# hkbharath/MARL-MASS

Hardware: AMD Instinct MI355X
Metric: agent-steps/sec (whole node), MASS CBF shield on, 65536 envs x 8 CAVs (higher is better)
Workload: dtype f64

## Files before the change

### marl-mass_amd/csrc/mm_kernels.hip

```cpp
#include <hip/hip_runtime.h>
#include <math.h>
#include <stdio.h>
#include <string.h>

#include <type_traits>

#include "mm_device.h"
#include "mm_div.h"
#include "mm_handle.h"
#define MM_COUNTS_FN __host__ __device__ inline
#include "../../include/mm_counts.h"
#include "../../include/mm_policy_wide.h"

using namespace mm;

struct DevCfg {
  int env_kind, shield, nsub, T, action_masking, auto_reset, obs_f64, N, E, debug_flags, n_hdv;
  double dt, collision_reward, high_speed_reward, headway_cost, headway_time, merging_lane_cost;
  double rs_lo, rs_hi, eta, tau;
  double inv_dt, rs_span, rs_ispan, rs_span2, rs_ispan2;
  int agent_reward;
  int steer_vel;
  int *err;
  int traffic_density, mixed_traffic, num_cav;
// ... 311 lines not shown
    const double a_lc = clipd(acc, kLcMinAcc, kLcMaxAcc);
    v.act_acc = lc_vehicle ? a_lc : acc;
  } else {
  if (v.crashed) { v.act_steer = 0; st_t = 0; v.act_acc = -1.0 * v.v; }
  if (v.v > kMaxSpeed) v.act_acc = fmin(v.act_acc, 1.0 * (kMaxSpeed - v.v));
  else if (v.v < -kMaxSpeed) v.act_acc = fmax(v.act_acc, 1.0 * (kMaxSpeed - v.v));
  if (lc_vehicle) v.act_acc = clipd(v.act_acc, kLcMinAcc, kLcMaxAcc);
  }
}

template <bool SEL = false>
MM_DEV int corner_flags(double x, double y, double sh, double ch, int lane) {
  double cx = x + (kCornerLen * mmm_cos_sum(MMM_CORNER_SIN, MMM_CORNER_COS, sh, ch));
  double cyL = y - (kCornerLen * mmm_sin_sum(MMM_CORNER_SIN, MMM_CORNER_COS, sh, ch)) + 0.01;
  double cyR = y - (kCornerLen * mmm_sin_sum(-MMM_CORNER_SIN, MMM_CORNER_COS, sh, ch)) + 0.01;
  double s = cx - lane_sx(lane);
  if constexpr (SEL && kCornerSelects) {
    const bool kb = lane == MM_LANE_KB0;
    double sn = 0.0;
    if (kb) sn = sin_f<true>(kSinePuls * s + kSinePhase);
    const double off = kb ? kSineAmp * sn : 0.0;
    const bool lon = (-kVehLength <= s) & (s < lane_len(lane) + kVehLength);
    const double rL0 = cyL - lane_sy(lane), rR0 = cyR - lane_sy(lane);
    const double rL = kb ? rL0 - off : rL0, rR = kb ? rR0 - off : rR0;
    return (!((fabs(rL) <= kLaneWidth / 2 + 0) & lon) ? 1 : 0) | (!((fabs(rR) <= kLaneWidth / 2 + 0) & lon) ? 2 : 0);
  }
  double off = (lane == MM_LANE_KB0) ? kSineAmp * sin_f<SEL>(kSinePuls * s + kSinePhase) : 0.0;
  bool lon = (-kVehLength <= s && s < lane_len(lane) + kVehLength);
  double rL = cyL - lane_sy(lane), rR = cyR - lane_sy(lane);
  if (lane == MM_LANE_KB0) { rL = rL - off; rR = rR - off; }
  return (!(fabs(rL) <= kLaneWidth / 2 + 0 && lon) ? 1 : 0) | (!(fabs(rR) <= kLaneWidth / 2 + 0 && lon) ? 2 : 0);
}
MM_DEV int pose_code(int lane, int nl, int off) { return lane | nl << 3 | off << 6; }

struct Cand {
  double x, y, h, gvx, cpsi, spsi;
  int lane;
  int pk;
};
template <int KIND, bool SHIELDED, bool CORNERS = SHIELDED, bool GENERAL = true, bool SINE = false>
MM_DEV Cand predict(const Veh &v, double steer, double st_t, double sh, double ch, double dt, bool sv = false, double *sine_out = nullptr) {
  Cand c;
  double ht = st_t, sb, cb;
  if constexpr (GENERAL) {
    if (__any(sv || st_t != st_t)) {
      double s2, c2;
      mmm_sincos(sv ? v.sang : steer, &s2, &c2);
      if (sv || st_t != st_t) ht = 1.0 / 2 * (s2 / c2);
    }
  }
  mmm_slip_sincos(ht, &sb, &cb);
  double vx = v.v * mmm_cos_sum(sh, ch, sb, cb), vy = v.v * mmm_sin_sum(sh, ch, sb, cb);
  c.x = v.x + vx * dt;
  c.y = v.y + vy * dt;
  const double d_heading = MM_DIVC(v.v * sb, 2.5);
  c.h = v.h + (sv ? d_heading : d_heading * dt);
  mmm_sincos(c.h, &c.spsi, &c.cpsi);
  c.gvx = (KIND == MM_ENV_V1) ? mmm_cos_sum(c.spsi, c.cpsi, sb, cb) : 0.0;
  c.lane = closest_lane<SINE>(c.x, c.y, c.h, sine_out);
  c.pk = c.lane;
  if (SHIELDED) c.pk = pose_code(c.lane, next_lane(c.lane, c.x, c.y), CORNERS ? corner_flags<SINE>(c.x, c.y, c.spsi, c.cpsi, c.lane) : 0);
  return c;
}

MM_DEV int adj_pair(int l1, int l2) {
  return (l1 == MM_LANE_BC0 && l2 == MM_LANE_BC1) ? -1 : ((l1 == MM_LANE_BC1 && l2 == MM_LANE_BC0) ? 1 : 0);
}
MM_DEV int adj_lane(int l1, int nl1, int l2) {
  const int f = adj_pair(l1, l2);
  return f != 0 ? f : adj_pair(nl1, l2);
}
MM_DEV unsigned adj_row(int l1) { return l1 == MM_LANE_BC0 ? (3u << (2 * MM_LANE_BC1)) : (l1 == MM_LANE_BC1 ? (1u << (2 * MM_LANE_BC0)) : 0u); }
MM_DEV unsigned adj_col(int l2) { return l2 == MM_LANE_BC1 ? (3u << (2 * MM_LANE_BC0)) : (l2 == MM_LANE_BC0 ? (1u << (2 * MM_LANE_BC1)) : 0u); }

struct QpTrace {
  double rows, a, h0, h1, h2, h3, d, margin;
};

MM_DEV void init_vehicle(Veh &v) {
  v.lane = closest_lane(v.x, v.y, v.h);
  v.tlane = v.lane;
  v.act_steer = v.act_acc = 0;
  v.safe_steer = v.safe_acc = 0;
  if (v.kind == 2) {
    v.sidx = 0;
    v.tspeed = v.v;
    v.gvx = py_mod((v.x + v.y) * kPi, 1.0);
  } else {
    v.sidx = speed_to_index(v.v);
    v.tspeed = index_to_speed(v.sidx);
    v.gvx = __builtin_nan("");
  }
  v.h1x = v.h1vx = v.h2x = v.h2vx = 0;
  v.sang = 0;
// ... 27 lines not shown
  else if (a < n_cav + n_sh) { main_road = true; k = n_s + (a - n_cav); }
  else { main_road = false; k = n_m + (a - n_cav - n_sh); }
  int slots[6];
#pragma unroll
  for (int i = 0; i < 6; i++) slots[i] = (main_road ? 10 : 5) + 50 * i;
  int chosen = 0;
#pragma unroll
  for (int i = 0; i < 6; i++) {
    if (i <= k) {
      const uint32_t ri = main_road ? r[i] : r[6 + i];
      int j = i + (int)(((uint64_t)ri * (uint32_t)(6 - i)) >> 32);
      int si = slots[i], sj = 0;
#pragma unroll
      for (int q = 0; q < 6; q++) if (q == j) sj = slots[q];
#pragma unroll
      for (int q = 0; q < 6; q++) if (q == j) slots[q] = si;
      slots[i] = sj;
      if (i == k) chosen = sj;
    }
  }
  rng_block(seed, episode, 3u + (uint32_t)a, blk);
  double speed = u53(blk[0], blk[1]) * 2 + 25;
  double noise = u53(blk[2], blk[3]) * 8 - 4;
  v.x = chosen + noise;
  v.y = main_road ? 0.0 : 10.5;
  v.h = 0;
  v.v = speed;
  v.kind = a < n_cav ? 1 : 2;
  v.present = true;
  init_vehicle(v);
  return n_m;
}

template <int G, int KIND, bool LEND = false, bool SEL = kScanSelects>
MM_DEV void observe(const DevCfg &c, const Veh &v, int a, int gb, long long i, bool valid, void *obs,
                    uint8_t *avail, float *stage = nullptr, const double *sincos_h = nullptr) {
  constexpr int F = (KIND != MM_ENV_V0) ? 6 : 5;
  constexpr int S = 5 * F;
  const bool ctrl = kIdm<KIND> ? v.present : (v.present && v.kind != 2);
  float *sw;
  if constexpr (LEND) {
    sw = stage + (threadIdx.x >> 6) * (64 * S);
  } else {
    __shared__ float s_obs[4][64 * S];
    sw = s_obs[threadIdx.x >> 6];
  }
  static_assert(64 * S * sizeof(float) >= 5 * 64 * sizeof(double), "the mailbox must fit in the row staging");
  if (obs) {
    const int lane = lane_id();
    double sps, cps;
    if (sincos_h) { sps = sincos_h[0]; cps = sincos_h[1]; }
    else mmm_sincos(v.h, &sps, &cps);
    const double vx = v.v * cps, vy = v.v * sps;
    const double sx = lane_sx(v.lane);
    double *mb = (double *)sw;
    mb[0 * 64 + lane] = v.x; mb[1 * 64 + lane] = v.y; mb[2 * 64 + lane] = vx; mb[3 * 64 + lane] = vy;
    if (KIND != MM_ENV_V0) mb[4 * 64 + lane] = v.h;
    __builtin_amdgcn_fence(__ATOMIC_RELEASE, "wavefront");
    __builtin_amdgcn_wave_barrier();
    __builtin_amdgcn_fence(__ATOMIC_ACQUIRE, "wavefront");
    double key[G];
    key[0] = 0;
    for_partners<G>([&](auto mc) {
      constexpr int m = decltype(mc)::value;
      const int pl = plane<m, G>(lane, a);
      double px = mb[0 * 64 + pl], py = mb[1 * 64 + pl];
      bool pp = px_i<m, G>((int)v.present, a) != 0;
// ... 58 lines not shown
      put(0, ctrl ? 1.0 : 0.0);
#pragma unroll
      for (int f = 0; f < F - 1; f++) {
        if constexpr (SEL) { const double w = lmap(ego[f], f); put(1 + f, ctrl ? w : 0.0); }
        else put(1 + f, ctrl ? lmap(ego[f], f) : 0.0);
      }
#pragma unroll
      for (int q = 0; q < 4; q++) {
        bool hq;
        if constexpr (SEL) hq = ctrl & have[q];
        else hq = ctrl && have[q];
        put((q + 1) * F, hq ? 1.0 : 0.0);
#pragma unroll
        for (int f = 0; f < F - 1; f++) {
          if constexpr (SEL) { const double w = lmap(row[q][f], f); put((q + 1) * F + 1 + f, hq ? w : 0.0); }
          else put((q + 1) * F + 1 + f, hq ? lmap(row[q][f], f) : 0.0);
        }
      }
    };
    if (c.obs_f64) {
      if (valid) emit([&](int k, double val) { ((double *)obs)[i * (5 * F) + k] = val; });
    } else {
      const int slot = (lane / G) * c.N + a;
      if (valid) emit([&](int k, double val) { sw[slot * S + k] = (float)val; });
      __builtin_amdgcn_fence(__ATOMIC_RELEASE, "wavefront");
      __builtin_amdgcn_wave_barrier();
      __builtin_amdgcn_fence(__ATOMIC_ACQUIRE, "wavefront");
      const long long wave_lane0 = (long long)blockIdx.x * blockDim.x + threadIdx.x - lane;
      const long long e0 = kPow2<G> ? wave_lane0 / G : (wave_lane0 >> 6) * (64 / G);
      long long nenv = (long long)c.E - e0;
      nenv = nenv < 0 ? 0 : (nenv > 64 / G ? 64 / G : nenv);
      const int total = (int)nenv * c.N * S;
      float *dst = (float *)obs + e0 * c.N * S;
      if constexpr (S % 2 == 0) {
        for (int t = lane; t < total / 2; t += 64) ((float2 *)dst)[t] = ((const float2 *)sw)[t];
      } else {
        for (int t = lane; t < total; t += 64) dst[t] = sw[t];
      }
    }
  }
  unsigned bits = 0x1F;
  if (!kIdm<KIND> && c.action_masking) {
    unsigned mine = 0;
    if (ctrl) {
      mine = 1u << 1;
      if (v.lane == MM_LANE_BC1 && lane_reachable(MM_LANE_BC0, v.x, v.y)) mine |= 1u << 0;
      if (v.lane == MM_LANE_BC0 && lane_reachable(MM_LANE_BC1, v.x, v.y)) mine |= 1u << 2;
      if (v.sidx < 4) mine |= 1u << 3;
      if (v.sidx > 0) mine |= 1u << 4;
    }
    bits = 0;
#pragma unroll
    for (int k = 0; k < 5; k++)
      if (group_ballot<G>((mine >> k) & 1u, gb)) bits |= 1u << k;
  }
  if (valid && avail) {
#pragma unroll
    for (int k = 0; k < 5; k++) avail[i * 5 + k] = (!kIdm<KIND> && ctrl) ? (uint8_t)((bits >> k) & 1u) : (uint8_t)0;
  }
}

struct Body {
  bool present, is_object;
  double x, y, h, v, tspeed;
  int lane;
  double sh, ch, koff;
};
MM_DEV double desired_gap(const Body &ego, const Body &front) {
  constexpr double ab = 15.0;
  const double es = ego.sh, ec = ego.ch, fs = front.sh, fc = front.ch;
// ... 188 lines not shown
  o.us0 = us0; o.veto = veto; o.flags = fl;
  o.qt.rows = s.cadj ? 4 : 3; o.qt.a = s.g0; o.qt.h0 = r.h0; o.qt.h1 = s.h1; o.qt.h2 = s.h2; o.qt.h3 = r.h3; o.qt.d = d;
  o.qt.margin = fmin(fmin(s.hls_lona, inv_lona), fmin(s.hls_lonr, inv_lonr));
  return o;
}
template <bool MASS, bool PRE = false, bool IPM = false>
MM_DEV ShieldOut shield_dyn(const DevCfg &c, const Veh &v, const ShieldStatic &s, const Neigh &nb, bool run_qp = true) {
  const ShieldRows r = shield_rows<PRE>(c, s, nb);
  double d;
  bool optimal = true;
  if constexpr (IPM) {
    d = 0.0;
    if (run_qp) {
      double slack;
      int iters;
      optimal = mm_qp_ipm_cbf(s.g0, r.h0, s.h1, s.h2, r.h3, s.cadj ? 4 : 3, &d, &slack, &iters) != 0;
    }
  } else {
    d = qp_exact(s, r);
  }
  return shield_post<MASS>(c, v, s, r, d, optimal, IPM && run_qp);
}
template <bool MASS, bool PRE = false, bool IPM = false>
MM_DEV ShieldOut shield_eval(const DevCfg &c, const Veh &v, double cpsi, int pk_self, const Neigh &nb, bool run_qp = true) {
  const ShieldStatic s = shield_static<MASS>(c, v, cpsi, pk_self, nb);
  return shield_dyn<MASS, PRE, IPM>(c, v, s, nb, run_qp);
}

struct Rel {
  double key;
  int cls;
  bool cflag;
};
MM_DEV Rel relate(double ex, double ey, int epk, bool other, double ox, double oy, double oh, int opk, bool o_hdv = false) {
  const int elane = epk & 7, enl = (epk >> 3) & 7, olane = opk & 7, onl = (opk >> 3) & 7;
  Rel r;
  const double dx = ox - ex, dy = oy - ey;
  const bool close = other & ((dx * dx + dy * dy) < kT180);
  const double esx = lane_sx(elane);
  const double ld = (ox - esx) - (ex - esx);
  r.key = close ? fabs(ld) : INFINITY;
  const unsigned rowE = adj_row(elane), rowN = adj_row(enl);
  const unsigned nzE = (rowE | rowE >> 1) & 0x555u;
  const unsigned rowEN = rowE | (rowN & ~(nzE * 3u));
  const unsigned colE = adj_col(elane);
  const unsigned va_c = (rowEN >> (2 * olane)) & 3u;
  const unsigned g1 = (colE >> (2 * olane)) & 3u, g2 = (colE >> (2 * onl)) & 3u;
  const unsigned av_c = g1 != 0 ? g1 : g2;
  const bool head = (dy < 0) ? (oh > 0.037) : (oh < -0.037);
  const bool appr = (!(ld < 0)) & (fabs(dy) <= 3.5) & head;
  const bool adj = (!appr) & ((va_c | av_c) != 0);
  const bool same = (elane == olane) | (olane == enl);
  const bool twin = o_hdv & (!adj) & (elane == MM_LANE_AB0) & (olane == MM_LANE_KB0) & (ld >= 0);
  const bool lead = (!adj) & (!twin) & (same | appr) & (ld > 0);
  const int cls = adj ? ((ld < 0) ? 3 : 2) : (twin ? 4 : (lead ? 1 : 0));
  r.cls = close ? cls : 0;
  r.cflag = ((opk >> (((va_c == 3u) | (av_c == 1u)) ? 6 : 7)) & 1) != 0;
  return r;
}

MM_DEV void trace_status(double *t, long long A, const ShieldOut &o) {
  t[MM_T_STATUS * A] = (double)(MM_ST_RAN | (o.optimal ? MM_ST_IS_OPTIMAL : 0u) | (o.lon_safe ? MM_ST_IS_SAFE : 0u) |
                                (o.lon_invariant ? MM_ST_IS_INVARIANT : 0u) | (o.bounds ? MM_ST_QP_BOUNDS : 0u));
  t[MM_T_HEADWAY * A] = o.hw_num / o.hw_den;
}

#ifndef MM_SWEEP_GATE_T
#define MM_SWEEP_GATE_T 48
#endif
#ifndef MM_SWEEP_GATE_W
#define MM_SWEEP_GATE_W 8
#endif
#ifndef MM_SWEEP_SPEC_AT
#define MM_SWEEP_SPEC_AT 13
#endif
#ifndef MM_SWEEP_GATE_WU
#define MM_SWEEP_GATE_WU 3
#endif
template <int NV, bool MASS, bool MIXED = false>
__global__ __launch_bounds__(64, 1) void sweep_kernel(DevCfg c, DevState st, SweepBuf sb, int k, double *trace) {
  const long long A = st.A;
  enum { W_X = 0, W_Y, W_H, W_HX, W_GU, W_VX };
// ... 372 lines not shown
#endif
__global__ __launch_bounds__(MM_STEP_BLOCK, (SPLIT ? MM_SPLIT_WAVES : step_min_waves<G, SHIELD, MIXED>(IPM))) void step_kernel(DevCfg c, DevState st, const int32_t *__restrict__ actions,
                                                   MMStepOut out, double *metrics, SweepBuf sb, int kb, PoseBuf pb) {
  constexpr bool IDM = kIdm<KIND>;
  constexpr bool LC = (KIND == MM_ENV_V1) || IDM;
  constexpr bool SHIELDED = LC && (SHIELD != MM_SHIELD_NONE);
  static_assert(!IDM || (MIXED && SHIELD == MM_SHIELD_NONE && !IPM && !SPLIT), "hdv-v1: general unshielded kernels only");
  constexpr bool MASS = (SHIELD == MM_SHIELD_MASS);
  static_assert(!IPM || SHIELDED, "the IPM mode lives in shielded kernels");
  static_assert(!SPLIT || IPM, "the split form exists for the interior-point kernels");
#ifdef MM_SERIAL_ALL
  constexpr bool kSerialOnly = true || IPM;
#else
#ifdef MM_SERIAL_MASS
  constexpr bool kSerialOnly = MIXED || MASS || IPM;
#else
  constexpr bool kSerialOnly = MIXED;
#endif
#endif
  constexpr bool kSine = SHIELDED && !SPLIT && !MIXED && !IPM && !kSerialOnly && kPow2<G> && G <= 8;
  constexpr bool kScan = kScanSelects && !MIXED && !TRACE;
#ifndef MM_CARRY_POSE
#define MM_CARRY_POSE 1
#endif
  constexpr bool kCarry = kSine && MM_CARRY_POSE != 0;
#ifndef MM_PRIMARY_PRIOR
#define MM_PRIMARY_PRIOR 1
#endif
  constexpr bool kPrimary = kSine && !TRACE && kVetoPrior && MM_PRIMARY_PRIOR != 0;
#ifndef MM_SINE_CARRY
#define MM_SINE_CARRY 0
#endif
  constexpr bool kSineCarry = kPrimary && MM_SINE_CARRY != 0;
  constexpr bool kEarly = kSine && MM_EARLY_LOADS != 0;
  double car_sn = __builtin_nan("");
  (void)car_sn;
  static_assert(kPow2<G> || MM_STEP_BLOCK == 64, "rotation layouts: one wave per workgroup");
  const long long gtid = (long long)blockIdx.x * blockDim.x + threadIdx.x;
  constexpr int kTail = kPow2<G> ? 64 : (64 / G) * G;
  const bool tail = lane_id() >= kTail;
  const int gb = kPow2<G> ? (lane_id() & ~(G - 1)) : (tail ? kTail - G : lane_id() - lane_id() % G);
  const int a = kPow2<G> ? (int)(gtid % G) : lane_id() - gb;
  const long long e = kPow2<G> ? gtid / G : (tail ? (long long)st.E : (gtid >> 6) * (64 / G) + lane_id() / G);
  const bool valid = e < st.E && a < st.N;
  const long long i = e * st.N + a;
  const long long A = st.A;
  const double dt = c.dt;

#ifdef MM_STAMPS
  const unsigned long long _rec_t0 = __builtin_amdgcn_s_memtime(), _rec_rt0 = __builtin_amdgcn_s_memrealtime();
  unsigned long long _t_last = __builtin_amdgcn_s_memtime(), _t_acc = 0;
#endif
  Veh v;
  const bool sv = MIXED && KIND == MM_ENV_V1 && c.steer_vel != 0;
  int steps = 0, time = 0, n_merge = 0, episode = 0;
  int car_code = 0;
  long long car_kx = 0, car_ky = 0, car_kh = 0;
  double car_s = 0.0, car_c = 1.0;
  int act_raw = 1;
  (void)act_raw;
  if constexpr (kEarly) {
    if (valid) act_raw = actions[i];
    if (e < st.E) { n_merge = st.I[MM_E_N_MERGE * st.E + e]; episode = st.I[MM_E_EPISODE * st.E + e]; }
  }
  if constexpr (kCarry) {
    if (valid) {
      car_kx = __double_as_longlong(pb.F[PB_KX * A + i]); car_ky = __double_as_longlong(pb.F[PB_KY * A + i]);
      car_kh = __double_as_longlong(pb.F[PB_KH * A + i]);
      car_s = pb.F[PB_SIN * A + i]; car_c = pb.F[PB_COS * A + i]; car_code = pb.code[i];
    }
  }
  load_veh(st, i, valid, v, sv);
  if (e < st.E) {
    steps = st.I[MM_E_STEPS * st.E + e]; time = st.I[MM_E_TIME * st.E + e];
  }
  if (!MIXED && v.kind == 2) v.kind = 1;
  if (IDM && v.present) v.kind = 2;
  const bool hdv = MIXED && v.kind == 2;
  const bool ctrl = IDM ? v.present : (v.present && !hdv);
  const bool ctrl_x = IDM ? false : ctrl;
  int action;
  if constexpr (kEarly) action = ctrl ? act_raw : 1;
  else action = (!IDM && valid && ctrl) ? actions[i] : 1;
  if ((unsigned)action > 4u) {
    if (!SPLIT || kb == 0) atomicOr(c.err, MM_LATCH_BAD_ACTION);
    action = 1;
  }
  const unsigned present_bits = group_ballot<G>(v.present, gb);
  const unsigned ctrl_bits = group_ballot<G>(ctrl, gb);
  const int n_veh = __popc(present_bits), n_ctrl = __popc(ctrl_bits);
  if (!SPLIT || kb == 0) steps += 1;

  double cpsi = 1.0, spsi = 0.0;
  double st_t = __builtin_nan("");
  int pk_self = v.lane;
  bool carried = false;
  if constexpr (kCarry) {
    const bool hit = car_kx == __double_as_longlong(v.x) && car_ky == __double_as_longlong(v.y) && car_kh == __double_as_longlong(v.h) &&
                     (car_code >> 8) == ((kPoseWritten >> 8) | (MASS ? 1 : 0)) && (car_code & 7) == v.lane;
    carried = !__any(v.present && !hit);
    if (carried && v.present) { spsi = car_s; cpsi = car_c; pk_self = car_code & 0xFF; }
  }
  if (!carried) {
    if (v.present) mmm_sincos(v.h, &spsi, &cpsi);
    if (SHIELDED && v.present) pk_self = pose_code(v.lane, next_lane(v.lane, v.x, v.y), MASS ? corner_flags<kSine>(v.x, v.y, spsi, cpsi, v.lane) : 0);
  }

  enum { C_B = 0, C_H1X = 8, C_H1VX, C_H2X, C_H2VX, C_SSTEER, C_SACC, C_TSPEED, C_A = 15, C_GU0 = 23, C_GU1 = 24, C_PRE = 25, C_MSGW = 29 };
  constexpr bool kMailbox = G <= 8 || !kPow2<G>;
  constexpr bool kPackMsg = !kPow2<G>;
  constexpr int kColdB = kMailbox ? (kPackMsg ? 29 : 30) : 25;
  constexpr bool kRoomy = false;
  constexpr int C_CPSI = kColdB + G - 1, C_GVX = C_CPSI + 1;
  constexpr int kColdN = !SHIELDED ? 15 : (kSerialOnly ? 23 : kColdB + G - 1 + (kRoomy ? 2 : 0));
  static_assert(kColdN * MM_STEP_BLOCK * 8 >= (MM_STEP_BLOCK / 64) * 64 * 30 * 4, "the obs staging must fit in the cold slots");
  __shared__ double s_cold[kColdN][MM_STEP_BLOCK];
  const int tid = threadIdx.x;
  auto cold_i = [&](int slot, int col) -> int & { return ((int *)&s_cold[slot][col])[0]; };
  if (LC) {
    s_cold[C_H1X][tid] = v.h1x; s_cold[C_H1VX][tid] = v.h1vx; s_cold[C_H2X][tid] = v.h2x; s_cold[C_H2VX][tid] = v.h2vx;
    s_cold[C_SSTEER][tid] = v.safe_steer; s_cold[C_SACC][tid] = v.safe_acc;
  }
  s_cold[C_TSPEED][tid] = v.tspeed;
  if constexpr (kEarly) {
    static_assert(kMailbox && !kPackMsg, "the high words of the pose-code and rank-word slots must be free");
    ((int *)&s_cold[C_PRE + 3][tid])[1] = n_merge; ((int *)&s_cold[C_MSGW][tid])[1] = episode;
  }
  if constexpr (kRoomy) { s_cold[C_CPSI][tid] = cpsi; s_cold[C_GVX][tid] = v.gvx; }
  auto CPSI = [&]() -> double { if constexpr (kRoomy) return s_cold[C_CPSI][tid]; else return cpsi; };
  auto GVX = [&]() -> double { if constexpr (kRoomy) return s_cold[C_GVX][tid]; else return v.gvx; };
  bool env_active = IDM ? n_veh > 0 : n_ctrl > 0;
  if constexpr (SPLIT) {
    if (kb > 0) env_active = e < st.E && sb.envf[e] != 0;
  }
  STAMP(0);
  const int k_lo = SPLIT ? (kb > 0 ? kb - 1 : 0) : 0, k_hi = SPLIT ? (kb < c.nsub ? kb : c.nsub - 1) : c.nsub - 1;
  for (int k = k_lo; k <= k_hi; k++) {
    const bool head = !SPLIT || k == kb, tail = !SPLIT || k != kb;
    const bool live = env_active && v.present;
    QpTrace qt = {0, __builtin_nan(""), __builtin_nan(""), __builtin_nan(""), __builtin_nan(""),
                  __builtin_nan(""), __builtin_nan(""), __builtin_nan("")};
    int rank = 0;
    if ((SHIELDED || MIXED) && head) {
      for_partners<G>([&](auto mc) {
        constexpr int m = decltype(mc)::value;
        double px = px_d<m, G>(v.x, a);
        bool pp = px_i<m, G>((int)live, a) != 0;
        if constexpr (kScan) rank += (pp & ((px > v.x) | ((px == v.x) & (pidx<m, G>(a) < a)))) ? 1 : 0;
        else rank += (pp && (px > v.x || (px == v.x && pidx<m, G>(a) < a))) ? 1 : 0;
      });
    }
    if (head) v.tspeed = s_cold[C_TSPEED][tid];
    if (live && !hdv && head) {
      if (time % c.nsub == 0) hl_act<KIND>(v, action);
    }
    const int tl_pre = v.tlane;
    if (live && !hdv && head) controlled_act<!MIXED && !kPrimary, kSine>(v, -1, sv, st_t);
    if (head) s_cold[C_TSPEED][tid] = v.tspeed;
    if constexpr (MIXED) { STAMP(1); }
    if constexpr (MIXED) {
      if (head && __any(hdv && live)) {
        const bool acting = hdv && live && !v.crashed;
        double koff = 0.0, koff_obst = 0.0;
        if (__any(acting && v.lane == MM_LANE_KB0)) {
          koff = kSineAmp * mmm_sin(kSinePuls * (v.x - lane_sx(MM_LANE_KB0)) + kSinePhase);
          koff_obst = kSineAmp * mmm_sin(kSinePuls * (kObstX - lane_sx(MM_LANE_KB0)) + kSinePhase);
        }
        Body self = {true, false, v.x, v.y, v.h, v.v, v.tspeed, v.lane, spsi, cpsi, koff};
        const double s_me = v.x - lane_sx(v.lane);
        NbSel n0 = {0, 0, -1, -1}, n1 = {0, 0, -1, -1};
        const LaneFrame lf0 = lane_frame(v.lane);
        if (acting && lane_after_end(v.tlane, v.x)) v.tlane = next_lane(v.tlane, v.x, v.y);
        const int my_tl = v.tlane;
        const bool lc_branch = v.lane != my_tl;
        const bool same_road = lane_road(v.lane) == lane_road(my_tl);
        const bool timer_due = !lc_branch && (1.0 < v.gvx);
        const int side = v.lane == MM_LANE_BC0 ? MM_LANE_BC1 : (v.lane == MM_LANE_BC1 ? MM_LANE_BC0 : -1);
        const bool try_mobil = acting && timer_due && side >= 0 && lane_reachable(side < 0 ? 0 : side, v.x, v.y);
        const int sl = side < 0 ? 0 : side;
        const double s_side = v.x - lane_sx(sl);
        const LaneFrame lf1 = lane_frame(sl);
        unsigned abort_mask = 0;
        for_partners<G>([&](auto mc) {
          constexpr int m = decltype(mc)::value;
          const int p = pidx<m, G>(a);
          const bool bp = px_i<m, G>((int)live, a) != 0;
          const double bx = px_d<m, G>(v.x, a), by = px_d<m, G>(v.y, a), bk = px_d<m, G>(koff, a);
          if (acting) {
            neighbour_update(lf0, s_me, bp, bx, by, bk, p, n0);
            if (try_mobil) neighbour_update(lf1, s_side, bp, bx, by, bk, p, n1);
// ... 49 lines not shown
          const bool changed = nxt != tl_post;
          tl_post = nxt;
          if (!__any(changed)) break;
        }
        if constexpr (MIXED) { STAMP(5); }
        if (acting) {
          v.tlane = tl_post;
          v.act_acc = clipd(acc_f0, -6.0, 6.0);
        }
      }
      if (head && live && (!hdv || !v.crashed)) steer_lane(v, sv && !hdv, st_t);
      if (head && hdv && live) v.gvx += dt;
    }
    bool first_B = false;
    if constexpr (kPrimary) {
      static_assert(!MIXED && !SPLIT, "kPrimary: no HDVs, no steer_vel, every launch a whole step");
      first_B = (c.debug_flags & 1) == 0 && live && v.hist_len >= 2 && (v.tlane != v.lane || v.crashed) && !(v.flags & MM_FLAG_IS_LC_SAFE);
      if (live) {
        const int tl_1 = v.tlane + (first_B ? v.lane - v.tlane : 0);
        const double steer = steering_control<kSine, kSineCarry>(v.x, v.y, v.h, v.v, tl_1, st_t, car_sn);
        v.act_steer = clipd(steer, -kPi / 3, kPi / 3);
        const double steer_1 = v.act_steer, st_t_1 = st_t;
        clip_actions<kSine>(v, LC, st_t);
        if (first_B) { v.act_steer = steer_1; st_t = st_t_1; }
      }
    } else {
      if (live && head) clip_actions<kSine>(v, LC && !hdv, st_t);
    }
    STAMP(1);
    Cand cA;
    memset(&cA, 0, sizeof cA);
    const bool shield_on = SHIELDED && live && !hdv && v.hist_len >= 2;
    if constexpr (kSineCarry) car_sn = __builtin_nan("");
    if (live && head) cA = predict<KIND, SHIELDED, MASS, MIXED, kSine>(v, v.act_steer, st_t, spsi, cpsi, dt, sv && !hdv, kSineCarry ? &car_sn : nullptr);
    auto park = [&](auto base_c, const Cand &cc, double steer) {
      constexpr int base = decltype(base_c)::value;
      if constexpr (SHIELDED) {
        s_cold[base + 0][tid] = cc.x; s_cold[base + 1][tid] = cc.y; s_cold[base + 2][tid] = cc.h;
        cold_i(base + 3, tid) = cc.pk; s_cold[base + 4][tid] = cc.cpsi; s_cold[base + 5][tid] = steer;
        s_cold[base + 6][tid] = cc.gvx; s_cold[base + 7][tid] = cc.spsi;
      }
    };
    auto park_at = [&](int base, const Cand &cc, double steer) {
      s_cold[base + 0][tid] = cc.x; s_cold[base + 1][tid] = cc.y; s_cold[base + 2][tid] = cc.h;
      cold_i(base + 3, tid) = cc.pk; s_cold[base + 4][tid] = cc.cpsi; s_cold[base + 5][tid] = steer;
      s_cold[base + 6][tid] = cc.gvx; s_cold[base + 7][tid] = cc.spsi;
    };
    if constexpr (kPrimary) park_at(first_B ? (int)C_B : (int)C_A, cA, v.act_steer);
    else if (head) park(std::integral_constant<int, C_A>{}, cA, v.act_steer);
    STAMP(2);
    const bool needB = SHIELDED && shield_on && (v.tlane != v.lane || v.crashed || sv);
    bool haveB = first_B, haveA = !first_B;
    (void)haveA;
    auto make_other = [&]() {
      if constexpr (kPrimary) {
        const bool mk_A = !haveA;
        if (mk_A || (needB && !haveB)) {
          double t_o;
          const int tl_o = v.lane + (mk_A ? v.tlane - v.lane : 0);
          double steer_o = steering_control<kSine>(v.x, v.y, v.h, v.v, tl_o, t_o);
          if (mk_A) {
            steer_o = clipd(steer_o, -kPi / 3, kPi / 3);
            if (v.crashed) { steer_o = 0; t_o = 0; }
          }
          park_at(mk_A ? (int)C_A : (int)C_B, predict<KIND, true, MASS, MIXED, kSine>(v, steer_o, t_o, spsi, cpsi, dt, false), steer_o);
          haveA = true; haveB = haveB || !mk_A;
        }
      }
    };
    auto make_B = [&]() {
      if constexpr (SHIELDED) {
        if (needB && !haveB) {
          double tB;
          double steerB = steering_control<kSine>(v.x, v.y, v.h, v.v, v.lane, tB);
          if (sv) steerB = steer_vel_command(steerB, v.sang);
          park(std::integral_constant<int, C_B>{}, predict<KIND, true, MASS, MIXED, kSine>(v, steerB, tB, spsi, CPSI(), dt, sv), steerB);
          haveB = true;
        }
      }
    };
    auto chosen = [&](bool useB) {
      if constexpr (!SHIELDED) {
        return cA;
      } else {
        const int base = useB ? C_B : C_A;
        Cand cc;
        cc.x = s_cold[base + 0][tid]; cc.y = s_cold[base + 1][tid]; cc.h = s_cold[base + 2][tid];
        cc.gvx = s_cold[base + 6][tid]; cc.cpsi = s_cold[base + 4][tid]; cc.spsi = s_cold[base + 7][tid];
        const int pk = cold_i(base + 3, tid);
        cc.pk = pk; cc.lane = pk & 7;
        return cc;
      }
    };
    if constexpr (SPLIT) {
      if (!head && live && valid) {
        v.act_acc = sw_f(sb, SW_ACCN, a, e);
        if (MIXED && hdv) {
          v.act_steer = sw_f(sb, SW_ASTEER, a, e);
          if (sw_i(sb, SW_RES, a, e) & 16) s_cold[C_H1X][tid] = sw_f(sb, SW_ACC, a, e);
        }
        s_cold[C_A + 0][tid] = sw_f(sb, SW_AX, a, e); s_cold[C_A + 1][tid] = sw_f(sb, SW_AY, a, e); s_cold[C_A + 2][tid] = sw_f(sb, SW_AH, a, e);
        cold_i(C_A + 3, tid) = sw_i(sb, SW_APK, a, e); s_cold[C_A + 4][tid] = sw_f(sb, SW_ACPSI, a, e); s_cold[C_A + 5][tid] = sw_f(sb, SW_ASTEER, a, e);
        s_cold[C_A + 6][tid] = sw_f(sb, SW_AGVX, a, e); s_cold[C_A + 7][tid] = sw_f(sb, SW_ASPSI, a, e);
        if (needB) {
          s_cold[C_B + 0][tid] = sw_f(sb, SW_BX, a, e); s_cold[C_B + 1][tid] = sw_f(sb, SW_BY, a, e); s_cold[C_B + 2][tid] = sw_f(sb, SW_BH, a, e);
          cold_i(C_B + 3, tid) = sw_i(sb, SW_BPK, a, e); s_cold[C_B + 4][tid] = sw_f(sb, SW_BCPSI, a, e); s_cold[C_B + 5][tid] = sw_f(sb, SW_BSTEER, a, e);
          s_cold[C_B + 6][tid] = sw_f(sb, SW_BGVX, a, e); s_cold[C_B + 7][tid] = sw_f(sb, SW_BSPSI, a, e);
          haveB = true;
        }
// ... 69 lines not shown
          if ((threadIdx.x & 63) == 13) _t_acc += 1 + (pass == 0 ? 1ull << 32 : 0ull);
#endif
#endif
          const double mine_gvx = s_cold[(use_B ? C_B : C_A) + 6][tid];
          const double h1vx_mine = s_cold[C_H1VX][tid];
          s_cold[C_GU0][tid] = slot_gu<MASS>(s_cold[C_H2VX][tid], MASS ? s_cold[C_SACC][tid] : kCbfAccLo, GVX(), dt);
          s_cold[C_GU1][tid] = slot_gu<MASS>(h1vx_mine, kCbfAccLo, mine_gvx, dt);
          if constexpr (kMailbox) {
            const int my_word = (live ? rank : 99) | (use_B ? 256 : 0);
            if constexpr (kPackMsg) ((int *)&s_cold[C_PRE + 3][tid])[1] = my_word;
            else cold_i(C_MSGW, tid) = my_word;
            __builtin_amdgcn_fence(__ATOMIC_RELEASE, "wavefront");
            __builtin_amdgcn_wave_barrier();
            __builtin_amdgcn_fence(__ATOMIC_ACQUIRE, "wavefront");
          }
          Cand mine;
          if constexpr (!kMailbox) mine = chosen(use_B);
          double k_ol = INFINITY, k_oa = INFINITY, k_oar = INFINITY;
          int j_ol = -1, j_oa = -1, j_oar = -1;
          for_partners<G>([&](auto mc) {
            constexpr int m = decltype(mc)::value;
            const int p = pidx<m, G>(a);
            int p_rank, opk;
            double ox, oy, oh;
            bool i_first;
            if constexpr (kMailbox) {
              const int pl = plane<m, G>(tid, a);
              int pw;
              if constexpr (kPackMsg) pw = ((const int *)&s_cold[C_PRE + 3][pl])[1];
              else pw = cold_i(C_MSGW, pl);
              p_rank = pw & 255;
              i_first = live && rank < p_rank;
              const int pb = (!i_first && p_rank < 99) ? ((pw & 256) ? (int)C_B : (int)C_A) : (int)C_PRE;
              ox = s_cold[pb + 0][pl]; oy = s_cold[pb + 1][pl]; oh = s_cold[pb + 2][pl];
              opk = cold_i(pb + 3, pl) | (p_rank < 99 ? 256 : 0);
            } else {
              p_rank = dppx_i<m>(live ? rank : 99);
              i_first = live && rank < p_rank;
              const double sx_ = i_first ? mine.x : v.x, sy_ = i_first ? mine.y : v.y, sh_ = i_first ? mine.h : v.h;
              const int spk = i_first ? mine.pk : pk_self;
              ox = dppx_d<m>(sx_); oy = dppx_d<m>(sy_); oh = dppx_d<m>(sh_);
              opk = dppx_i<m>(spk | (int)live << 8);
            }
            const bool o_first = !i_first && p_rank < 99;
            const Rel r = relate(v.x, v.y, pk_self, ((opk >> 8) & 1) != 0, ox, oy, oh, opk);
            if constexpr (count5) s_cold[kColdB + m - 1][tid] = r.key;
            const bool b_ol = (r.cls == 1) & ((r.key < k_ol) | ((r.key == k_ol) & (p < (j_ol & 15))));
            const bool b_oa = (r.cls == 2) & ((r.key < k_oa) | ((r.key == k_oa) & (p < (j_oa & 15))));
            const bool b_oar = (r.cls == 3) & ((r.key < k_oar) | ((r.key == k_oar) & (p < (j_oar & 15))));
            const int pf = p | (o_first ? 16 : 0) | (r.cflag ? 32 : 0);
            k_ol = b_ol ? r.key : k_ol; j_ol = b_ol ? pf : j_ol;
            k_oa = b_oa ? r.key : k_oa; j_oa = b_oa ? pf : j_oa;
            k_oar = b_oar ? r.key : k_oar; j_oar = b_oar ? pf : j_oar;
          });
          const bool ol_first = j_ol >= 0 && (j_ol & 16), oa_first = j_oa >= 0 && (j_oa & 16), oar_stepped = j_oar >= 0 && (j_oar & 16);
          const bool cadj = j_oa >= 0 && (j_oa & 32);
          j_ol = j_ol < 0 ? -1 : (j_ol & 15); j_oa = j_oa < 0 ? -1 : (j_oa & 15); j_oar = j_oar < 0 ? -1 : (j_oar & 15);
          STAMP(3);
          Neigh nb;
          memset(&nb, 0, sizeof nb);
          nb.has_ol = j_ol >= 0; nb.has_oa = j_oa >= 0; nb.has_oar = j_oar >= 0;
          if constexpr (count5) {
            int pos_ol = 0, pos_oa = 0, pos_oar = 0;
#pragma unroll
            for (int m = 1; m < G; m++) {
              const int p = pidx_rt<G>(a, m);
              const double km = s_cold[kColdB + m - 1][tid];
              pos_ol += (km < k_ol || (km == k_ol && p < j_ol)) ? 1 : 0;
              pos_oa += (km < k_oa || (km == k_oa && p < j_oa)) ? 1 : 0;
              pos_oar += (km < k_oar || (km == k_oar && p < j_oar)) ? 1 : 0;
            }
            nb.has_ol = nb.has_ol && pos_ol < 5;
            nb.has_oa = nb.has_oa && pos_oa < 5;
            nb.has_oar = nb.has_oar && pos_oar < 5;
          }
          nb.constrain_adj = MASS && nb.has_oa && cadj;
          if constexpr (SPLIT) {
            if (valid && shield_on)
              sw_i(sb, SW_CLS, a, e) = (j_ol & 15) | (j_oa & 15) << 4 | (j_oar & 15) << 8 | (nb.has_ol ? 1 << 12 : 0) | (nb.has_oa ? 1 << 13 : 0) |
                                       (nb.has_oar ? 1 << 14 : 0) | (nb.constrain_adj ? 1 << 15 : 0);
            break;
          }
          __builtin_amdgcn_fence(__ATOMIC_RELEASE, "wavefront");
          __builtin_amdgcn_wave_barrier();
          __builtin_amdgcn_fence(__ATOMIC_ACQUIRE, "wavefront");
          const int t_ol = tid - a + (j_ol < 0 ? a : j_ol), t_oa = tid - a + (j_oa < 0 ? a : j_oa);
          nb.ol_x = s_cold[ol_first ? C_H1X : C_H2X][t_ol]; nb.ol_gu = s_cold[ol_first ? C_GU1 : C_GU0][t_ol];
          nb.oa_x = s_cold[oa_first ? C_H1X : C_H2X][t_oa]; nb.oa_gu = s_cold[oa_first ? C_GU1 : C_GU0][t_oa];
          const int src_ol = gb + (j_ol < 0 ? 0 : j_ol), src_oa = gb + (j_oa < 0 ? 0 : j_oa), src_oar = gb + (j_oar < 0 ? 0 : j_oar);
          const double cpsi_now = CPSI();
          nb.oar_x = shfl_d(v.x, src_oar); nb.oar_vx = shfl_d(v.v * cpsi_now, src_oar);
          bool ol_dyn = MASS && nb.has_ol && ol_first, oa_dyn = MASS && nb.has_oa && oa_first;
          {
            unsigned rep = obstacle_override<MASS>(nb, v.x, v.y);
            if (rep & 1u) ol_dyn = false;
            if (rep & 2u) oa_dyn = false;
          }
          irregular = irregular || (shield_on && nb.has_oar && oar_stepped);
          double acc_cur = shield_on ? 0.0 : v.act_acc;
          if constexpr (kRoomy) v.gvx = GVX();
          const ShieldStatic ss = shield_static<MASS>(c, v, cpsi_now, pk_self, nb);
          if constexpr (IPM) {
            bool fin = !shield_on, run = false, sing = false;
            bool late = false, late_opt = false;
            const bool slow_lc = MASS && (v.hl == 2 || v.hl == 0) && v.v < kStoppingSpeed;
            MMQpState q;
            q.x0 = 0.0; q.m4 = 0; q.iters = 0;
            bool more = true;
            for (int trip = 0; more; trip++) {
              if (trip > (MM_QP_MAXITERS + 2) * (G + 1)) { atomicOr(c.err, MM_LATCH_INTERNAL); break; }
              MMQpRes rs;
              bool done_now = late, opt = late_opt;
              late = false;
              if (run) {
                const int stop = mm_qp_top(&q, &rs);
                if (stop || sing) { run = false; done_now = true; opt = stop == 1 && !sing; }
              }
              if (__any(done_now)) {
                if (done_now) {
                  double us0 = ss.u0 + q.x0;
                  if (MASS && slow_lc) us0 = shield_post<MASS>(c, v, ss, shield_rows<true>(c, ss, nb), q.x0, opt, true).us0;
                  acc_cur = div_c(us0 - ss.evx, dt, c.inv_dt);
                  fin = true;
                  qc_d = q.x0; qc_meta = (ss.cadj ? 4 : 3) | (opt ? 8 : 0);
                }
              }
              bool ready = shield_on && !fin && !run;
              double da = 0.0, db = 0.0;
              if (MASS) {
                const double gu_cur = slot_gu<true>(h1vx_mine, acc_cur, mine_gvx, dt);
                da = shfl_d(gu_cur, src_ol); db = shfl_d(gu_cur, src_oa);
                const unsigned long long fm = __ballot(fin);
                ready = ready && (!ol_dyn || ((fm >> src_ol) & 1ull)) && (!oa_dyn || ((fm >> src_oa) & 1ull));
              }
// ... 172 lines not shown
            if constexpr (G >= 8) red(std::integral_constant<int, 7>{});
            if constexpr (G >= 16) red(std::integral_constant<int, 8>{});
          } else {
            auto ring = [&](auto mc) {
              constexpr int off = decltype(mc)::value;
              if constexpr (off < G) {
                const unsigned o = (unsigned)px_i<off, G>((int)w, a);
                const unsigned m0 = min(w & 0x3FFu, o & 0x3FFu), m1 = min((w >> 10) & 0x3FFu, (o >> 10) & 0x3FFu),
                               m2 = min((w >> 20) & 0x3FFu, (o >> 20) & 0x3FFu);
                w = m0 | m1 << 10 | m2 << 20;
                if (MIXED) f_tw = min(f_tw, (unsigned)px_i<off, G>((int)f_tw, a));
              }
            };
            ring(std::integral_constant<int, 1>{}); ring(std::integral_constant<int, 2>{});
            ring(std::integral_constant<int, 4>{}); ring(std::integral_constant<int, 8>{});
          }
          f_ol = w & 0x3FFu; f_oa = (w >> 10) & 0x3FFu; f_oar = (w >> 20) & 0x3FFu;
          const bool has_tw = MIXED && f_tw != none;
          if (has_tw) f_oa = f_tw & ~1u;
          Neigh nb;
          nb.has_ol = f_ol != none; nb.has_oa = f_oa != none; nb.has_oar = f_oar != none;
          const int s_ol = gb + (nb.has_ol ? (int)((f_ol >> 1) & 15u) : 0);
          const int s_oa = gb + (nb.has_oa ? (int)((f_oa >> 1) & 15u) : 0);
          const int s_oar = gb + (nb.has_oar ? (int)((f_oar >> 1) & 15u) : 0);
          nb.ol_x = shfl_d(whx, s_ol); nb.ol_gu = shfl_d(wgu, s_ol);
          nb.oa_x = shfl_d(whx, s_oa); nb.oa_gu = shfl_d(wgu, s_oa);
          nb.ol_vx = nb.oa_vx = nb.ol_acc = nb.ol_g = nb.oa_acc = nb.oa_g = 0;
          nb.oar_x = shfl_d(wx, s_oar); nb.oar_vx = shfl_d(wvx, s_oar);
          nb.constrain_adj = MASS && nb.has_oa && (f_oa & 1u);
          bool hss_collab = false;
          if (has_tw) { nb.constrain_adj = MASS; hss_collab = !MASS; }
          obstacle_override<MASS>(nb, v.x, v.y);
          const bool mine = has && a == ai && shield_on;
          ShieldOut s1 = shield_eval<MASS, true, IPM>(c, v, cpsi, pk_self, nb, mine);
          if (hss_collab) s1.flags |= MM_FLAG_IS_COLLABORATING;
          if (IPM && mine && s1.bounds) atomicOr(c.err, MM_LATCH_QP_BOUNDS);
          if (mine) {
            new_acc = s1.acc; veto = s1.veto; new_flags = s1.flags; qt = s1.qt;
            if (TRACE) trace_status(out.trace + (long long)k * MM_T_COUNT * A + i, A, s1);
            use_B = veto && needB;
            const Cand cc = chosen(use_B);
            double nv = v.v + new_acc * dt;
            nv = nv > 0 ? nv : 0;
            wx = cc.x; wy = cc.y; wh = cc.h; wg = cc.gvx; wacc = new_acc; wvx = nv * cc.cpsi;
            whx = s_cold[C_H1X][tid]; whvx = s_cold[C_H1VX][tid]; wpk = cc.pk;
            wgu = slot_gu<MASS>(whvx, MASS ? wacc : kCbfAccLo, wg, dt);
          }
        }
        if (MIXED && hdv && twin_shift != 0 && w_stepped) s_cold[C_H1X][tid] = whx;
      }
     }
    }
    STAMP(6);
    CAND_COUNT(MM_CS_PRIOR_HELD, st_prior && use_B);
    CAND_COUNT(MM_CS_PRIOR_LIFTED, st_prior && !use_B);
    if (SPLIT && SHIELDED && out.trace && live && tail && !shield_on) {
      out.trace[(long long)k * MM_T_COUNT * A + i + MM_T_QP_ROWS * A] = 0;
    }
    if (!SPLIT && SHIELDED && TRACE && live) {
      double *t = out.trace + (long long)k * MM_T_COUNT * A + i;
      t[MM_T_QP_ROWS * A] = qt.rows; t[MM_T_QP_A * A] = qt.a;
      t[MM_T_QP_H0 * A] = qt.h0; t[MM_T_QP_H1 * A] = qt.h1; t[MM_T_QP_H2 * A] = qt.h2;
      t[MM_T_QP_H3 * A] = qt.h3; t[MM_T_QP_D * A] = qt.d; t[MM_T_LC_MARGIN * A] = qt.margin;
    }
    if (tail) {
    if constexpr (kSineCarry) {
      if (!(live && use_B == first_B)) car_sn = __builtin_nan("");
// ... 289 lines not shown
        row[ln] = acc;
      }
    }
  }
  STAMP(15);
  if constexpr (kCarry) { car_s = spsi; car_c = cpsi; }
  if (c.auto_reset && done) {
    const uint64_t seed = st.seeds[e];
    Veh nv;
    memset(&nv, 0, sizeof nv);
    int nm = 0;
    int nc = n_ctrl, nh = n_veh - n_ctrl;
    if constexpr (IDM) { nc = 0; nh = n_veh; }
    episode_counts<KIND>(c, seed, (uint32_t)episode, nc, nh);
    const bool spawn = valid && (c.traffic_density > 0 ? a < nc + nh : v.present);
    if (spawn) nm = spawn_vehicle(nv, a, nc, nh, seed, (uint32_t)episode);
    if (c.traffic_density > 0 && valid) {
      if (!spawn) {
        if (v.present) {
          Veh z;
          memset(&z, 0, sizeof z);
          store_veh(st, i, z, true);
        }
        v.present = false; v.kind = 0;
      }
      st.B[MM_B_KIND * A + i] = spawn ? (uint8_t)nv.kind : (uint8_t)0;
    }
    if (spawn) {
      v = nv;
      spsi = 0.0; cpsi = 1.0;
      if constexpr (kCarry) {
        mmm_sincos(v.h, &car_s, &car_c);
        pk_self = pose_code(v.lane, next_lane(v.lane, v.x, v.y), MASS ? corner_flags<kSine>(v.x, v.y, car_s, car_c, v.lane) : 0);
      }
      s_cold[C_H1X][tid] = v.h1x; s_cold[C_H1VX][tid] = v.h1vx; s_cold[C_H2X][tid] = v.h2x; s_cold[C_H2VX][tid] = v.h2vx;
      s_cold[C_SSTEER][tid] = v.safe_steer; s_cold[C_SACC][tid] = v.safe_acc; s_cold[C_TSPEED][tid] = v.tspeed;
    }
    n_merge = shfl_i(nm, gb);
    steps = 0; time = 0; episode += 1;
  }
  if (valid && v.present) {
    if (LC) {
      v.h1x = s_cold[C_H1X][tid]; v.h1vx = s_cold[C_H1VX][tid]; v.h2x = s_cold[C_H2X][tid]; v.h2vx = s_cold[C_H2VX][tid];
      if (!hdv) { v.safe_steer = s_cold[C_SSTEER][tid]; v.safe_acc = s_cold[C_SACC][tid]; }
    }
    v.tspeed = s_cold[C_TSPEED][tid];
    store_veh(st, i, v, sv);
    if constexpr (kCarry) {
      pb.F[PB_KX * A + i] = v.x; pb.F[PB_KY * A + i] = v.y; pb.F[PB_KH * A + i] = v.h;
      pb.F[PB_SIN * A + i] = car_s; pb.F[PB_COS * A + i] = car_c;
      pb.code[i] = (pk_self & 0xFF) | (MASS ? 0x100 : 0) | kPoseWritten;
    }
  }
  if (e < st.E && a == 0) {
    st.I[MM_E_STEPS * st.E + e] = steps; st.I[MM_E_TIME * st.E + e] = time;
    st.I[MM_E_N_MERGE * st.E + e] = n_merge; st.I[MM_E_EPISODE * st.E + e] = episode;
  }
  STAMP(11);
  __syncthreads();
  STAMP(14);
  const double sc_h[2] = {spsi, cpsi};
  observe<G, KIND, true, kScan>(c, v, a, gb, i, valid, out.obs, out.action_mask, (float *)&s_cold[0][0], sc_h);
  STAMP(12);
#ifdef MM_STAMPS
  {
    const long long wv = gtid >> 6;
    if ((threadIdx.x & 63) < 16 && wv < MM_STAMP_WAVES) g_stamps_w[wv * 16 + (threadIdx.x & 63)] += _t_acc;
    else if ((threadIdx.x & 63) < 32 && wv < MM_STAMP_WAVES) g_stamps_c[wv * 16 + (threadIdx.x & 63) - 16] += _t_acc;
    if (wv < MM_REC_WAVES) {
      unsigned long long *rec = g_wave_rec + wv * MM_REC_WORDS;
      const int respawned = __popcll(__ballot(c.auto_reset && done && a == 0 && e < st.E));
      if ((threadIdx.x & 63) < 32) rec[MM_REC_SLOTS + (threadIdx.x & 63)] = _t_acc;
      if ((threadIdx.x & 63) == 0) {
        const unsigned hw = __builtin_amdgcn_s_getreg(4 | (31 << 11)), xcc = __builtin_amdgcn_s_getreg(20 | (31 << 11));
        rec[MM_REC_BEGIN] = _rec_t0; rec[MM_REC_RT_BEGIN] = _rec_rt0;
        rec[MM_REC_HW] = (unsigned long long)hw | (unsigned long long)xcc << 32;
        rec[MM_REC_RESPAWN] = (unsigned long long)respawned;
        rec[MM_REC_RT_END] = __builtin_amdgcn_s_memrealtime();
        rec[MM_REC_END] = __builtin_amdgcn_s_memtime();
      }
    }
  }
#endif
}

template <int G, int KIND>
__global__ __launch_bounds__(256) void reset_kernel(DevCfg c, DevState st, int mode, const uint8_t *env_mask,
                                                    const uint64_t *seeds_in, void *obs, uint8_t *avail) {
  const long long gtid = (long long)blockIdx.x * blockDim.x + threadIdx.x;
  const long long e = gtid / G;
  const int a = (int)(gtid % G);
  const int gb = lane_id() & ~(G - 1);
  const bool valid = e < st.E && a < st.N;
  const long long i = e * st.N + a;
  const bool selected = e < st.E && mode != 2 && (!env_mask || env_mask[e]);
// ... 1183 lines not shown
```

Before: 2.600 billion.

## Pack heading-sign bits into pose code, widen obs copy, branch-free action select

Three separate changes. First, the heading-threshold sign is encoded as two extra bits in the pose code, so the neighbour relate step no longer needs to load the other vehicle's heading from shared memory. Second, the observation copy from LDS staging to global uses unrolled float4 loads and stores when a wave's env block is full and aligned, with the old float2 loop kept as fallback. Third, the high-level and controlled action updates run unconditionally on a copy and are merged back with selects, trading extra work on idle lanes for less divergence.

Measured after the change: 2.640 billion, median of 6. 1.5% higher.

```diff
diff --git a/marl-mass_amd/csrc/mm_kernels.hip b/marl-mass_amd/csrc/mm_kernels.hip
--- a/marl-mass_amd/csrc/mm_kernels.hip
+++ b/marl-mass_amd/csrc/mm_kernels.hip
@@ -367,13 +367,19 @@
   return (!(fabs(rL) <= kLaneWidth / 2 + 0 && lon) ? 1 : 0) | (!(fabs(rR) <= kLaneWidth / 2 + 0 && lon) ? 2 : 0);
 }
 MM_DEV int pose_code(int lane, int nl, int off) { return lane | nl << 3 | off << 6; }
+#ifndef MM_POSE_HBITS
+#define MM_POSE_HBITS 1
+#endif
+constexpr bool kPoseHBits = MM_POSE_HBITS != 0;
+constexpr int kPoseHPos = 0x200, kPoseHNeg = 0x400;
+MM_DEV int pose_hbits(double h) { return ((h > 0.037) ? kPoseHPos : 0) | ((h < -0.037) ? kPoseHNeg : 0); }
 
 struct Cand {
   double x, y, h, gvx, cpsi, spsi;
   int lane;
   int pk;
 };
-template <int KIND, bool SHIELDED, bool CORNERS = SHIELDED, bool GENERAL = true, bool SINE = false>
+template <int KIND, bool SHIELDED, bool CORNERS = SHIELDED, bool GENERAL = true, bool SINE = false, bool HB = false>
 MM_DEV Cand predict(const Veh &v, double steer, double st_t, double sh, double ch, double dt, bool sv = false, double *sine_out = nullptr) {
   Cand c;
   double ht = st_t, sb, cb;
@@ -395,6 +401,7 @@
   c.lane = closest_lane<SINE>(c.x, c.y, c.h, sine_out);
   c.pk = c.lane;
   if (SHIELDED) c.pk = pose_code(c.lane, next_lane(c.lane, c.x, c.y), CORNERS ? corner_flags<SINE>(c.x, c.y, c.spsi, c.cpsi, c.lane) : 0);
+  if constexpr (HB) c.pk |= pose_hbits(c.h);
   return c;
 }
 
@@ -488,7 +495,11 @@
   return n_m;
 }
 
-template <int G, int KIND, bool LEND = false, bool SEL = kScanSelects>
+#ifndef MM_OBS_WIDE
+#define MM_OBS_WIDE 1
+#endif
+constexpr bool kObsWide = MM_OBS_WIDE != 0;
+template <int G, int KIND, bool LEND = false, bool SEL = kScanSelects, bool WIDE = false>
 MM_DEV void observe(const DevCfg &c, const Veh &v, int a, int gb, long long i, bool valid, void *obs,
                     uint8_t *avail, float *stage = nullptr, const double *sincos_h = nullptr) {
   constexpr int F = (KIND != MM_ENV_V0) ? 6 : 5;
@@ -613,10 +624,32 @@
       nenv = nenv < 0 ? 0 : (nenv > 64 / G ? 64 / G : nenv);
       const int total = (int)nenv * c.N * S;
       float *dst = (float *)obs + e0 * c.N * S;
-      if constexpr (S % 2 == 0) {
-        for (int t = lane; t < total / 2; t += 64) ((float2 *)dst)[t] = ((const float2 *)sw)[t];
+      auto copy_loop = [&]() {
+        if constexpr (S % 2 == 0) {
+          for (int t = lane; t < total / 2; t += 64) ((float2 *)dst)[t] = ((const float2 *)sw)[t];
+        } else {
+          for (int t = lane; t < total; t += 64) dst[t] = sw[t];
+        }
+      };
+      if constexpr (WIDE && LEND && S % 2 == 0 && (64 / G) * G * S % 4 == 0) {
+        constexpr int kFull4 = (64 / G) * G * S / 4, kTrips = (kFull4 + 63) / 64;
+        if (nenv == 64 / G && c.N == G && ((uintptr_t)dst & 15) == 0) {
+          float4 q[kTrips];
+#pragma unroll
+          for (int j = 0; j < kTrips; j++) {
+            const int t = lane + 64 * j;
+            q[j] = ((const float4 *)sw)[(64 * (j + 1) <= kFull4 || t < kFull4) ? t : lane];
+          }
+#pragma unroll
+          for (int j = 0; j < kTrips; j++) {
+            const int t = lane + 64 * j;
+            if (64 * (j + 1) <= kFull4 || t < kFull4) ((float4 *)dst)[t] = q[j];
+          }
+        } else {
+          copy_loop();
+        }
       } else {
-        for (int t = lane; t < total; t += 64) dst[t] = sw[t];
+        copy_loop();
       }
     }
   }
@@ -871,6 +904,7 @@
   int cls;
   bool cflag;
 };
+template <bool HB = false>
 MM_DEV Rel relate(double ex, double ey, int epk, bool other, double ox, double oy, double oh, int opk, bool o_hdv = false) {
   const int elane = epk & 7, enl = (epk >> 3) & 7, olane = opk & 7, onl = (opk >> 3) & 7;
   Rel r;
@@ -886,7 +920,9 @@
   const unsigned va_c = (rowEN >> (2 * olane)) & 3u;
   const unsigned g1 = (colE >> (2 * olane)) & 3u, g2 = (colE >> (2 * onl)) & 3u;
   const unsigned av_c = g1 != 0 ? g1 : g2;
-  const bool head = (dy < 0) ? (oh > 0.037) : (oh < -0.037);
+  bool head;
+  if constexpr (HB) head = (opk & ((dy < 0) ? kPoseHPos : kPoseHNeg)) != 0;
+  else head = (dy < 0) ? (oh > 0.037) : (oh < -0.037);
   const bool appr = (!(ld < 0)) & (fabs(dy) <= 3.5) & head;
   const bool adj = (!appr) & ((va_c | av_c) != 0);
   const bool same = (elane == olane) | (olane == enl);
@@ -1325,7 +1361,13 @@
 #define MM_SINE_CARRY 0
 #endif
   constexpr bool kSineCarry = kPrimary && MM_SINE_CARRY != 0;
+#ifndef MM_ACT_FRAME
+#define MM_ACT_FRAME 1
+#endif
+  constexpr bool kActSel = kPrimary && MM_ACT_FRAME != 0;
   constexpr bool kEarly = kSine && MM_EARLY_LOADS != 0;
+  constexpr bool kHBits = kSine && !TRACE && kPoseHBits;
+  constexpr bool kWideObs = kSine && !TRACE && kObsWide;
   double car_sn = __builtin_nan("");
   (void)car_sn;
   static_assert(kPow2<G> || MM_STEP_BLOCK == 64, "rotation layouts: one wave per workgroup");
@@ -1392,11 +1434,12 @@
     const bool hit = car_kx == __double_as_longlong(v.x) && car_ky == __double_as_longlong(v.y) && car_kh == __double_as_longlong(v.h) &&
                      (car_code >> 8) == ((kPoseWritten >> 8) | (MASS ? 1 : 0)) && (car_code & 7) == v.lane;
     carried = !__any(v.present && !hit);
-    if (carried && v.present) { spsi = car_s; cpsi = car_c; pk_self = car_code & 0xFF; }
+    if (carried && v.present) { spsi = car_s; cpsi = car_c; pk_self = (car_code & 0xFF) | (kHBits ? pose_hbits(v.h) : 0); }
   }
   if (!carried) {
     if (v.present) mmm_sincos(v.h, &spsi, &cpsi);
     if (SHIELDED && v.present) pk_self = pose_code(v.lane, next_lane(v.lane, v.x, v.y), MASS ? corner_flags<kSine>(v.x, v.y, spsi, cpsi, v.lane) : 0);
+    if constexpr (kHBits) { if (v.present) pk_self |= pose_hbits(v.h); }
   }
 
   enum { C_B = 0, C_H1X = 8, C_H1VX, C_H2X, C_H2VX, C_SSTEER, C_SACC, C_TSPEED, C_A = 15, C_GU0 = 23, C_GU1 = 24, C_PRE = 25, C_MSGW = 29 };
@@ -1407,7 +1450,7 @@
   constexpr int C_CPSI = kColdB + G - 1, C_GVX = C_CPSI + 1;
   constexpr int kColdN = !SHIELDED ? 15 : (kSerialOnly ? 23 : kColdB + G - 1 + (kRoomy ? 2 : 0));
   static_assert(kColdN * MM_STEP_BLOCK * 8 >= (MM_STEP_BLOCK / 64) * 64 * 30 * 4, "the obs staging must fit in the cold slots");
-  __shared__ double s_cold[kColdN][MM_STEP_BLOCK];
+  __shared__ alignas(kWideObs ? 16 : 8) double s_cold[kColdN][MM_STEP_BLOCK];
   const int tid = threadIdx.x;
   auto cold_i = [&](int slot, int col) -> int & { return ((int *)&s_cold[slot][col])[0]; };
   if (LC) {
@@ -1444,11 +1487,21 @@
       });
     }
     if (head) v.tspeed = s_cold[C_TSPEED][tid];
-    if (live && !hdv && head) {
-      if (time % c.nsub == 0) hl_act<KIND>(v, action);
+    if constexpr (kActSel) {
+      Veh w = v;
+      if (time % c.nsub == 0) hl_act<KIND>(w, action);
+      controlled_act<false, kSine>(w, -1, sv, st_t);
+      v.hl = live ? w.hl : v.hl; v.sidx = live ? w.sidx : v.sidx; v.tspeed = live ? w.tspeed : v.tspeed;
+      v.tlane = live ? w.tlane : v.tlane; v.act_acc = live ? w.act_acc : v.act_acc;
+    } else {
+      if (live && !hdv && head) {
+        if (time % c.nsub == 0) hl_act<KIND>(v, action);
+      }
     }
     const int tl_pre = v.tlane;
-    if (live && !hdv && head) controlled_act<!MIXED && !kPrimary, kSine>(v, -1, sv, st_t);
+    if constexpr (!kActSel) {
+      if (live && !hdv && head) controlled_act<!MIXED && !kPrimary, kSine>(v, -1, sv, st_t);
+    }
     if (head) s_cold[C_TSPEED][tid] = v.tspeed;
     if constexpr (MIXED) { STAMP(1); }
     if constexpr (MIXED) {
@@ -1564,7 +1617,7 @@
     memset(&cA, 0, sizeof cA);
     const bool shield_on = SHIELDED && live && !hdv && v.hist_len >= 2;
     if constexpr (kSineCarry) car_sn = __builtin_nan("");
-    if (live && head) cA = predict<KIND, SHIELDED, MASS, MIXED, kSine>(v, v.act_steer, st_t, spsi, cpsi, dt, sv && !hdv, kSineCarry ? &car_sn : nullptr);
+    if (live && head) cA = predict<KIND, SHIELDED, MASS, MIXED, kSine, kHBits>(v, v.act_steer, st_t, spsi, cpsi, dt, sv && !hdv, kSineCarry ? &car_sn : nullptr);
     auto park = [&](auto base_c, const Cand &cc, double steer) {
       constexpr int base = decltype(base_c)::value;
       if constexpr (SHIELDED) {
@@ -1595,7 +1648,7 @@
             steer_o = clipd(steer_o, -kPi / 3, kPi / 3);
             if (v.crashed) { steer_o = 0; t_o = 0; }
           }
-          park_at(mk_A ? (int)C_A : (int)C_B, predict<KIND, true, MASS, MIXED, kSine>(v, steer_o, t_o, spsi, cpsi, dt, false), steer_o);
+          park_at(mk_A ? (int)C_A : (int)C_B, predict<KIND, true, MASS, MIXED, kSine, kHBits>(v, steer_o, t_o, spsi, cpsi, dt, false), steer_o);
           haveA = true; haveB = haveB || !mk_A;
         }
       }
@@ -1606,7 +1659,7 @@
           double tB;
           double steerB = steering_control<kSine>(v.x, v.y, v.h, v.v, v.lane, tB);
           if (sv) steerB = steer_vel_command(steerB, v.sang);
-          park(std::integral_constant<int, C_B>{}, predict<KIND, true, MASS, MIXED, kSine>(v, steerB, tB, spsi, CPSI(), dt, sv), steerB);
+          park(std::integral_constant<int, C_B>{}, predict<KIND, true, MASS, MIXED, kSine, kHBits>(v, steerB, tB, spsi, CPSI(), dt, sv), steerB);
           haveB = true;
         }
       }
@@ -1742,7 +1795,9 @@
               p_rank = pw & 255;
               i_first = live && rank < p_rank;
               const int pb = (!i_first && p_rank < 99) ? ((pw & 256) ? (int)C_B : (int)C_A) : (int)C_PRE;
-              ox = s_cold[pb + 0][pl]; oy = s_cold[pb + 1][pl]; oh = s_cold[pb + 2][pl];
+              ox = s_cold[pb + 0][pl]; oy = s_cold[pb + 1][pl];
+              if constexpr (kHBits) oh = 0.0;
+              else oh = s_cold[pb + 2][pl];
               opk = cold_i(pb + 3, pl) | (p_rank < 99 ? 256 : 0);
             } else {
               p_rank = dppx_i<m>(live ? rank : 99);
@@ -1753,7 +1808,7 @@
               opk = dppx_i<m>(spk | (int)live << 8);
             }
             const bool o_first = !i_first && p_rank < 99;
-            const Rel r = relate(v.x, v.y, pk_self, ((opk >> 8) & 1) != 0, ox, oy, oh, opk);
+            const Rel r = relate<kHBits && kMailbox>(v.x, v.y, pk_self, ((opk >> 8) & 1) != 0, ox, oy, oh, opk);
             if constexpr (count5) s_cold[kColdB + m - 1][tid] = r.key;
             const bool b_ol = (r.cls == 1) & ((r.key < k_ol) | ((r.key == k_ol) & (p < (j_ol & 15))));
             const bool b_oa = (r.cls == 2) & ((r.key < k_oa) | ((r.key == k_oa) & (p < (j_oa & 15))));
@@ -1809,7 +1864,7 @@
           irregular = irregular || (shield_on && nb.has_oar && oar_stepped);
           double acc_cur = shield_on ? 0.0 : v.act_acc;
           if constexpr (kRoomy) v.gvx = GVX();
-          const ShieldStatic ss = shield_static<MASS>(c, v, cpsi_now, pk_self, nb);
+          const ShieldStatic ss = shield_static<MASS>(c, v, cpsi_now, kHBits ? pk_self & 0xFF : pk_self, nb);
           if constexpr (IPM) {
             bool fin = !shield_on, run = false, sing = false;
             bool late = false, late_opt = false;
@@ -2048,7 +2103,7 @@
           if (has_tw) { nb.constrain_adj = MASS; hss_collab = !MASS; }
           obstacle_override<MASS>(nb, v.x, v.y);
           const bool mine = has && a == ai && shield_on;
-          ShieldOut s1 = shield_eval<MASS, true, IPM>(c, v, cpsi, pk_self, nb, mine);
+          ShieldOut s1 = shield_eval<MASS, true, IPM>(c, v, cpsi, kHBits ? pk_self & 0xFF : pk_self, nb, mine);
           if (hss_collab) s1.flags |= MM_FLAG_IS_COLLABORATING;
           if (IPM && mine && s1.bounds) atomicOr(c.err, MM_LATCH_QP_BOUNDS);
           if (mine) {
@@ -2404,6 +2459,7 @@
       if constexpr (kCarry) {
         mmm_sincos(v.h, &car_s, &car_c);
         pk_self = pose_code(v.lane, next_lane(v.lane, v.x, v.y), MASS ? corner_flags<kSine>(v.x, v.y, car_s, car_c, v.lane) : 0);
+        if constexpr (kHBits) pk_self |= pose_hbits(v.h);
       }
       s_cold[C_H1X][tid] = v.h1x; s_cold[C_H1VX][tid] = v.h1vx; s_cold[C_H2X][tid] = v.h2x; s_cold[C_H2VX][tid] = v.h2vx;
       s_cold[C_SSTEER][tid] = v.safe_steer; s_cold[C_SACC][tid] = v.safe_acc; s_cold[C_TSPEED][tid] = v.tspeed;
@@ -2432,7 +2488,7 @@
   __syncthreads();
   STAMP(14);
   const double sc_h[2] = {spsi, cpsi};
-  observe<G, KIND, true, kScan>(c, v, a, gb, i, valid, out.obs, out.action_mask, (float *)&s_cold[0][0], sc_h);
+  observe<G, KIND, true, kScan, kWideObs>(c, v, a, gb, i, valid, out.obs, out.action_mask, (float *)&s_cold[0][0], sc_h);
   STAMP(12);
 #ifdef MM_STAMPS
   {
```
